# revdotcom/paper_accurate_fast_cheap

Measured on AMD Instinct MI355X. Metric: audio-sec/sec (1/RTF) GigaSpeech long-form encode, higher is better.
Workload: dtype f32+bf16-slot

## Files before the change

### paper_accurate_fast_cheap_amd/csrc/glue.hip

```cpp
#include <stdlib.h>

#include <type_traits>

#include "pafc_common.h"
#include "../../include/pafc_encoder_ops.h"

namespace pafc {

struct SplitBf16 {};
template <> struct Elem<SplitBf16> {
    __device__ static __forceinline__ float round(float v) { return v; }
};

namespace {

constexpr int VEC = 8;
constexpr int MAXIT = 2;

__device__ __forceinline__ void store8_split(bf16_t *hi_p, bf16_t *lo_p, const float *f) {
    float lo[VEC];
#pragma unroll
    for (int e = 0; e < VEC; ++e) lo[e] = f[e] - round_bf16(f[e]);
    store8<bf16_t>(hi_p, f);
    store8<bf16_t>(lo_p, lo);
// ... 137 lines not shown

template <typename ET>
__global__ __launch_bounds__(256) void tmix_shift_mix_kernel(int T, int C, long rows, int ndir, int rev0,
                                                             const ET *__restrict__ x, const ET *__restrict__ maa0,
                                                             const ET *__restrict__ maa1, ET *__restrict__ out,
                                                             const ET *__restrict__ prev) {
    const long gid = (long)blockIdx.x * 256 + threadIdx.x;
    const int cpr = C / VEC;
    const long row = gid / cpr;
    if (row >= rows) return;
    const int c = (int)(gid % cpr) * VEC;
    const int t = (int)(row % T);
    float xc[VEC], xp[VEC], xn[VEC];
    load8<ET>(x + row * C + c, xc);
#pragma unroll
    for (int e = 0; e < VEC; ++e) { xp[e] = 0.f; xn[e] = 0.f; }
    if (t > 0) load8<ET>(x + (row - 1) * C + c, xp);
    else if (prev) load8<ET>(prev + (row / T) * C + c, xp);
    if (t < T - 1) load8<ET>(x + (row + 1) * C + c, xn);
    for (int d = 0; d < ndir; ++d) {
        const bool rev = (d == 0) ? (rev0 != 0) : true;
        float m[VEC], o[VEC];
        load8<ET>((d == 0 ? maa0 : maa1) + c, m);
#pragma unroll
        for (int e = 0; e < VEC; ++e) {
            const float xx = Elem<ET>::round((rev ? xn[e] : xp[e]) - xc[e]);
            o[e] = Elem<ET>::round(xc[e] + Elem<ET>::round(xx * m[e]));
        }
        store8<ET>(out + ((size_t)d * rows + row) * C + c, o);
    }
}

template <typename ET>
__global__ __launch_bounds__(256) void tmix_mix4_kernel(int T, int C, long rows, int ndir, int rev0,
                                                        const ET *__restrict__ x, const ET *__restrict__ m,
                                                        const ET *__restrict__ maa, ET *__restrict__ z) {
    const long gid = (long)blockIdx.x * 256 + threadIdx.x;
    const int cpr = C / VEC;
    const long row = gid / cpr;
    if (row >= rows) return;
    const int c = (int)(gid % cpr) * VEC;
    const int t = (int)(row % T);
    float xc[VEC], xp[VEC], xn[VEC];
    load8<ET>(x + row * C + c, xc);
#pragma unroll
    for (int e = 0; e < VEC; ++e) { xp[e] = 0.f; xn[e] = 0.f; }
    if (t > 0) load8<ET>(x + (row - 1) * C + c, xp);
    if (t < T - 1) load8<ET>(x + (row + 1) * C + c, xn);
    for (int d = 0; d < ndir; ++d) {
        const bool rev = (d == 0) ? (rev0 != 0) : true;
        float xx[VEC];
#pragma unroll
        for (int e = 0; e < VEC; ++e) xx[e] = Elem<ET>::round((rev ? xn[e] : xp[e]) - xc[e]);
#pragma unroll
        for (int q = 0; q < 4; ++q) {
            float mv[VEC], av[VEC], o[VEC];
            load8<ET>(m + (((size_t)d * 4 + q) * rows + row) * C + c, mv);
            load8<ET>(maa + ((size_t)d * 4 + q) * C + c, av);
#pragma unroll
            for (int e = 0; e < VEC; ++e)
                o[e] = Elem<ET>::round(xc[e] + Elem<ET>::round(xx[e] * Elem<ET>::round(av[e] + mv[e])));
            store8<ET>(z + (((size_t)q * ndir + d) * rows + row) * C + c, o);
        }
    }
}

template <bool LDSW, bool FULLROW = false>
__global__ __launch_bounds__(256) void tmix_lora_mix4_kernel(int T, int C, long rows, int ndir, int rev0,
                                                             const bf16_t *__restrict__ x, const bf16_t *__restrict__ t,
                                                             const bf16_t *__restrict__ w2t,
                                                             const bf16_t *__restrict__ maa, bf16_t *__restrict__ z,
                                                             const bf16_t *__restrict__ prev) {
    const int lane = threadIdx.x & 63, wave = threadIdx.x >> 6;
    const int r16 = lane & 15, qq = lane >> 4;
    const long row = ((long)blockIdx.x * 4 + wave) * 16 + r16;
    const long rowc = row < rows ? row : rows - 1;
    const int tt = (int)(rowc % T);
    const f32x4 zero = {0.f, 0.f, 0.f, 0.f};
    constexpr int LDZ = 64 + 8;
    __shared__ __attribute__((aligned(16))) bf16_t s_z[4][16][LDZ];
    __shared__ __attribute__((aligned(16))) bf16_t s_w2[LDSW ? 2 : 1][LDSW ? 4 : 1][LDSW ? 64 : 1][32];
    if constexpr (LDSW) {
        for (int i = threadIdx.x; i < ndir * 4 * 64 * 4; i += 256) {
            const int ck = i & 3, col = (i >> 2) & 63, dq = i >> 8;
            *reinterpret_cast<uint4 *>(&s_w2[0][0][0][0] + ((size_t)dq * 64 + col) * 32 + 8 * ck) =
                *reinterpret_cast<const uint4 *>(w2t + ((size_t)dq * C + blockIdx.y * 64 + col) * 32 + 8 * ck);
        }
        __syncthreads();
    }
    for (int d = 0; d < ndir; ++d) {
        const bool rev = (d == 0) ? (rev0 != 0) : true;
        const bool in_seq = rev ? (tt < T - 1) : (tt > 0);
        const bool has_nb = in_seq || (prev != nullptr && !rev);
        const bf16_t *nbrow = in_seq ? x + (rev ? rowc + 1 : rowc - 1) * C : (has_nb ? prev + (rowc / T) * C : x + rowc * C);
        uint4 tb[4];
#pragma unroll
        for (int q = 0; q < 4; ++q)
            tb[q] = *reinterpret_cast<const uint4 *>(t + ((size_t)d * rows + rowc) * 128 + 32 * q + 8 * qq);
        float xc[2][VEC], xx[2][VEC];
#pragma unroll
        for (int cbi = 0; cbi < 2; ++cbi) {
            const int col = (blockIdx.y * 2 + cbi) * 32 + 8 * qq;
            float xn[VEC];
            load8<bf16_t>(x + rowc * C + col, xc[cbi]);
            load8<bf16_t>(nbrow + col, xn);
#pragma unroll
            for (int e = 0; e < VEC; ++e) xx[cbi][e] = round_bf16((has_nb ? xn[e] : 0.f) - xc[cbi][e]);
        }
#pragma unroll
        for (int q = 0; q < 4; ++q) {
#pragma unroll
            for (int cbi = 0; cbi < 2; ++cbi) {
                const int cb = blockIdx.y * 2 + cbi;
                const int col = cb * 32 + 8 * qq;
                const int colA = cb * 32 + 8 * (r16 >> 2) + (r16 & 3);
                uint4 a1, a2;
                if constexpr (LDSW) {
                    const int colL = colA - blockIdx.y * 64;
                    a1 = *reinterpret_cast<const uint4 *>(&s_w2[d][q][colL][8 * qq]);
                    a2 = *reinterpret_cast<const uint4 *>(&s_w2[d][q][colL + 4][8 * qq]);
                } else {
                    const bf16_t *wq = w2t + ((size_t)(d * 4 + q) * C) * 32 + 8 * qq;
                    a1 = *reinterpret_cast<const uint4 *>(wq + (size_t)colA * 32);
                    a2 = *reinterpret_cast<const uint4 *>(wq + (size_t)(colA + 4) * 32);
                }
                const f32x4 m1 = mfma_bf16_packed(a1, tb[q], zero);
                const f32x4 m2 = mfma_bf16_packed(a2, tb[q], zero);
                float av[VEC], o[VEC];
                load8<bf16_t>(maa + ((size_t)d * 4 + q) * C + col, av);
#pragma unroll
                for (int e = 0; e < VEC; ++e) {
                    const float mv = round_bf16(e < 4 ? m1[e] : m2[e - 4]);
                    o[e] = round_bf16(xc[cbi][e] + round_bf16(xx[cbi][e] * round_bf16(av[e] + mv)));
                }
                store8<bf16_t>(&s_z[wave][r16][cbi * 32 + 8 * qq], o);
            }
            __builtin_amdgcn_fence(__ATOMIC_RELEASE, "wavefront");
            __builtin_amdgcn_wave_barrier();
#pragma unroll
            for (int half = 0; half < 2; ++half) {
                const int rr = half * 8 + (lane >> 3), cc = (lane & 7) * 8;
                const long orow = ((long)blockIdx.x * 4 + wave) * 16 + rr;
                if (orow < rows)
                    *reinterpret_cast<uint4 *>(z + (((size_t)q * ndir + d) * rows + orow) * C + blockIdx.y * 64 + cc) =
                        *reinterpret_cast<const uint4 *>(&s_z[wave][rr][cc]);
            }
            __builtin_amdgcn_fence(__ATOMIC_RELEASE, "wavefront");
            __builtin_amdgcn_wave_barrier();
        }
    }
}


template <int NW, int WCOLS>
__global__ __launch_bounds__(NW * 64) void tmix_lora_mix4_ws_kernel(int T, int C, long rows, int ndir, int rev0,
                                                                const bf16_t *__restrict__ x, const bf16_t *__restrict__ t,
                                                                const bf16_t *__restrict__ w2t,
                                                                const bf16_t *__restrict__ maa, bf16_t *__restrict__ z,
                                                                const bf16_t *__restrict__ prev) {
    const int lane = threadIdx.x & 63, wave = threadIdx.x >> 6;
    const int r16 = lane & 15, qq = lane >> 4;
    constexpr int WROWS = NW / WCOLS;
    const int cy = blockIdx.y * WCOLS + wave % WCOLS, d = blockIdx.z;
    const int wrow = wave / WCOLS;
    const bool rev = (d == 0) ? (rev0 != 0) : true;
    const f32x4 zero = {0.f, 0.f, 0.f, 0.f};
    constexpr int LDZ = 64 + 8;
    __shared__ __attribute__((aligned(16))) bf16_t s_z[NW][16][LDZ];
    const int colslot = 8 * (r16 >> 2) + (r16 & 3);
    uint4 a1[4][2], a2[4][2], av[4][2];
#pragma unroll
    for (int q = 0; q < 4; ++q)
#pragma unroll
        for (int cbi = 0; cbi < 2; ++cbi) {
            const int cb = cy * 2 + cbi;
            const bf16_t *wq = w2t + ((size_t)(d * 4 + q) * C + cb * 32 + colslot) * 32 + 8 * qq;
            a1[q][cbi] = *reinterpret_cast<const uint4 *>(wq);
            a2[q][cbi] = *reinterpret_cast<const uint4 *>(wq + 4 * 32);
            av[q][cbi] = *reinterpret_cast<const uint4 *>(maa + ((size_t)d * 4 + q) * C + cb * 32 + 8 * qq);
        }
    const long ntiles = (rows + 15) / 16;
    for (long tile = (long)blockIdx.x * WROWS + wrow; tile < ntiles; tile += (long)gridDim.x * WROWS) {
        const long row = tile * 16 + r16;
        const long rowc = row < rows ? row : rows - 1;
        const int tt = (int)(rowc % T);
        const bool in_seq = rev ? (tt < T - 1) : (tt > 0);
        const bool has_nb = in_seq || (prev != nullptr && !rev);
        const bf16_t *nbrow = in_seq ? x + (rev ? rowc + 1 : rowc - 1) * C : (has_nb ? prev + (rowc / T) * C : x + rowc * C);
        uint4 tb[4];
#pragma unroll
        for (int q = 0; q < 4; ++q)
            tb[q] = *reinterpret_cast<const uint4 *>(t + ((size_t)d * rows + rowc) * 128 + 32 * q + 8 * qq);
        float xc[2][VEC], xx[2][VEC];
#pragma unroll
        for (int cbi = 0; cbi < 2; ++cbi) {
            const int col = (cy * 2 + cbi) * 32 + 8 * qq;
            float xn[VEC];
            load8<bf16_t>(x + rowc * C + col, xc[cbi]);
            load8<bf16_t>(nbrow + col, xn);
#pragma unroll
            for (int e = 0; e < VEC; ++e) xx[cbi][e] = round_bf16((has_nb ? xn[e] : 0.f) - xc[cbi][e]);
        }
#pragma unroll
        for (int q = 0; q < 4; ++q) {
#pragma unroll
            for (int cbi = 0; cbi < 2; ++cbi) {
                const f32x4 m1 = mfma_bf16_packed(a1[q][cbi], tb[q], zero);
                const f32x4 m2 = mfma_bf16_packed(a2[q][cbi], tb[q], zero);
                const unsigned aw[4] = {av[q][cbi].x, av[q][cbi].y, av[q][cbi].z, av[q][cbi].w};
                float o[VEC];
#pragma unroll
                for (int e = 0; e < VEC; ++e) {
                    const float a = (e & 1) ? __uint_as_float(aw[e >> 1] & 0xffff0000u) : __uint_as_float(aw[e >> 1] << 16);
                    const float mv = round_bf16(e < 4 ? m1[e] : m2[e - 4]);
                    o[e] = round_bf16(xc[cbi][e] + round_bf16(xx[cbi][e] * round_bf16(a + mv)));
                }
                store8<bf16_t>(&s_z[wave][r16][cbi * 32 + 8 * qq], o);
            }
            __builtin_amdgcn_fence(__ATOMIC_RELEASE, "wavefront");
            __builtin_amdgcn_wave_barrier();
#pragma unroll
            for (int half = 0; half < 2; ++half) {
                const int rr = half * 8 + (lane >> 3), cc = (lane & 7) * 8;
                const long orow = tile * 16 + rr;
                if (orow < rows)
                    *reinterpret_cast<uint4 *>(z + (((size_t)q * ndir + d) * rows + orow) * C + cy * 64 + cc) =
                        *reinterpret_cast<const uint4 *>(&s_z[wave][rr][cc]);
            }
            __builtin_amdgcn_fence(__ATOMIC_RELEASE, "wavefront");
            __builtin_amdgcn_wave_barrier();
        }
    }
}

constexpr int DL_C = 512, DL_H = 64;
constexpr int DL_WAVES = 8;
__global__ __launch_bounds__(DL_WAVES * 64) void decay_lora_kernel(long rows, int ndir, const bf16_t *__restrict__ zw,
                                                                   const bf16_t *__restrict__ d1n,
                                                                   const bf16_t *__restrict__ d2n,
                                                                   const bf16_t *__restrict__ bias, bf16_t *__restrict__ wout) {
    constexpr int C = DL_C;
    const int lane = threadIdx.x & 63, wave = threadIdx.x >> 6;
    const int r16 = lane & 15, qq = lane >> 4;
    const f32x4 zero = {0.f, 0.f, 0.f, 0.f};
    constexpr int LDZ = 64 + 8;
    extern __shared__ __attribute__((aligned(16))) unsigned char dl_lds[];
    uint4 *s_d1 = reinterpret_cast<uint4 *>(dl_lds);
    uint4 *s_d2 = s_d1 + 16 * 4 * 64;
    bf16_t(*s_z)[16][LDZ] = reinterpret_cast<bf16_t(*)[16][LDZ]>(s_d2 + 16 * 2 * 2 * 64);
    const int colslot = 8 * (r16 >> 2) + (r16 & 3);
    const long ntiles = (rows + 15) / 16;
    {
        const int d = blockIdx.y;
        for (int f = wave; f < 64; f += DL_WAVES) {
            const int ks = f >> 2, tau = f & 3;
            s_d1[f * 64 + lane] = *reinterpret_cast<const uint4 *>(d1n + ((size_t)d * DL_H + 16 * tau + r16) * C + 32 * ks + 8 * qq);
        }
        for (int f = wave; f < 64; f += DL_WAVES) {
            const int cb = f >> 2, a = (f >> 1) & 1, p = f & 1;
            const bf16_t *dq = d2n + ((size_t)d * C + cb * 32 + colslot + 4 * a) * DL_H + 32 * p + 4 * qq;
            const uint2 lo = *reinterpret_cast<const uint2 *>(dq), hi = *reinterpret_cast<const uint2 *>(dq + 16);
            s_d2[f * 64 + lane] = uint4{lo.x, lo.y, hi.x, hi.y};
        }
        __syncthreads();
        for (long tile = (long)blockIdx.x * DL_WAVES + wave; tile < ntiles; tile += (long)gridDim.x * DL_WAVES) {
            const long row = tile * 16 + r16;
            const long rowc = row < rows ? row : rows - 1;
            const bf16_t *zr = zw + ((size_t)d * rows + rowc) * C + 8 * qq;
            uint4 zf[16];
#pragma unroll
            for (int ks = 0; ks < 16; ++ks) zf[ks] = *reinterpret_cast<const uint4 *>(zr + 32 * ks);
            f32x4 acc1[4] = {zero, zero, zero, zero};
#pragma unroll
            for (int ks = 0; ks < 16; ++ks)
#pragma unroll
                for (int tau = 0; tau < 4; ++tau)
                    acc1[tau] = mfma_bf16_packed(s_d1[(ks * 4 + tau) * 64 + lane], zf[ks], acc1[tau]);
            u32x4 b2[2];
#pragma unroll
            for (int p = 0; p < 2; ++p) {
                float v[8];
#pragma unroll
                for (int e = 0; e < 8; ++e) v[e] = round_bf16(epilogue_act<2>(acc1[2 * p + (e >> 2)][e & 3]));
                b2[p] = u32x4{pack_bf16_exact(v[0], v[1]), pack_bf16_exact(v[2], v[3]),
                              pack_bf16_exact(v[4], v[5]), pack_bf16_exact(v[6], v[7])};
            }
            for (int cy = 0; cy < C / 64; ++cy) {
#pragma unroll
                for (int cbi = 0; cbi < 2; ++cbi) {
                    const int cb = cy * 2 + cbi;
                    f32x4 o[2];
#pragma unroll
                    for (int a = 0; a < 2; ++a) {
                        o[a] = mfma_bf16_packed(s_d2[((cb * 2 + a) * 2 + 0) * 64 + lane], b2[0], zero);
                        o[a] = mfma_bf16_packed(s_d2[((cb * 2 + a) * 2 + 1) * 64 + lane], b2[1], o[a]);
                    }
                    float ov[VEC];
#pragma unroll
                    for (int e = 0; e < VEC; ++e) ov[e] = e < 4 ? o[0][e] : o[1][e - 4];
                    if (bias) {
                        float bv[VEC];
                        load8<bf16_t>(bias + (size_t)d * C + cb * 32 + 8 * qq, bv);
#pragma unroll
                        for (int e = 0; e < VEC; ++e) ov[e] = bv[e] + round_bf16(ov[e]);
                    }
                    store8<bf16_t>(&s_z[wave][r16][cbi * 32 + 8 * qq], ov);
                }
                __builtin_amdgcn_fence(__ATOMIC_RELEASE, "wavefront");
                __builtin_amdgcn_wave_barrier();
#pragma unroll
                for (int half = 0; half < 2; ++half) {
                    const int rr = half * 8 + (lane >> 3), cc = (lane & 7) * 8;
                    const long orow = tile * 16 + rr;
                    if (orow < rows)
                        *reinterpret_cast<uint4 *>(wout + ((size_t)d * rows + orow) * C + cy * 64 + cc) =
                            *reinterpret_cast<const uint4 *>(&s_z[wave][rr][cc]);
                }
                __builtin_amdgcn_fence(__ATOMIC_RELEASE, "wavefront");
                __builtin_amdgcn_wave_barrier();
            }
        }
    }
}

constexpr int LD_C = 512, LD_N = 128;
template <int NW>
__global__ __launch_bounds__(NW * 64) void tmix_lora_down_kernel(int T, long rows, int rev0, const bf16_t *__restrict__ x,
                                                                       const bf16_t *__restrict__ maa_x,
                                                                       const bf16_t *__restrict__ w1n, bf16_t *__restrict__ tout,
                                                                       const bf16_t *__restrict__ prev) {
    constexpr int C = LD_C;
    const int lane = threadIdx.x & 63, wave = threadIdx.x >> 6;
    const int r16 = lane & 15, qq = lane >> 4;
    const f32x4 zero = {0.f, 0.f, 0.f, 0.f};
    extern __shared__ __attribute__((aligned(16))) unsigned char dl_lds[];
    uint4 *s_w1 = reinterpret_cast<uint4 *>(dl_lds);
    const int colslot = 8 * (r16 >> 2) + (r16 & 3);
    const int d = blockIdx.y;
    const bool rev = (d == 0) ? (rev0 != 0) : true;
    for (int f = wave; f < 128; f += NW) {
        const int ks = f >> 3, np = (f >> 1) & 3, a = f & 1;
        s_w1[f * 64 + lane] = *reinterpret_cast<const uint4 *>(w1n + ((size_t)d * LD_N + 32 * np + colslot + 4 * a) * C + 32 * ks + 8 * qq);
    }
    __syncthreads();
    const long ntiles = (rows + 15) / 16;
    for (long tile = (long)blockIdx.x * NW + wave; tile < ntiles; tile += (long)gridDim.x * NW) {
        const long row = tile * 16 + r16;
        const long rowc = row < rows ? row : rows - 1;
        const int tt = (int)(rowc % T);
        const bool in_seq = rev ? (tt < T - 1) : (tt > 0);
        const bool has_nb = in_seq || (prev != nullptr && !rev);
        const bf16_t *nbrow = in_seq ? x + (rev ? rowc + 1 : rowc - 1) * C : (has_nb ? prev + (rowc / T) * C : x + rowc * C);
        const bf16_t *xr = x + rowc * C + 8 * qq, *xnr = nbrow + 8 * qq, *mr = maa_x + (size_t)d * C + 8 * qq;
        f32x4 acc[4][2];
#pragma unroll
        for (int np = 0; np < 4; ++np) { acc[np][0] = zero; acc[np][1] = zero; }
#pragma unroll 1
        for (int kc = 0; kc < 16; kc += 4)
#pragma unroll
        for (int ks = kc; ks < kc + 4; ++ks) {
            float xc[VEC], xn[VEC], mm[VEC];
            load8<bf16_t>(xr + 32 * ks, xc);
            load8<bf16_t>(xnr + 32 * ks, xn);
            load8<bf16_t>(mr + 32 * ks, mm);
            float o[VEC];
#pragma unroll
            for (int e = 0; e < VEC; ++e) {
                const float xx = round_bf16((has_nb ? xn[e] : 0.f) - xc[e]);
                o[e] = xc[e] + round_bf16(xx * mm[e]);
            }
            const u32x4 bq = {pack_bf16_rne(o[0], o[1]), pack_bf16_rne(o[2], o[3]), pack_bf16_rne(o[4], o[5]),
                              pack_bf16_rne(o[6], o[7])};
            __builtin_amdgcn_s_setprio(1);
#pragma unroll
            for (int np = 0; np < 4; ++np)
#pragma unroll
                for (int a = 0; a < 2; ++a)
                    acc[np][a] = mfma_bf16_packed(s_w1[((ks * 4 + np) * 2 + a) * 64 + lane], bq, acc[np][a]);
            __builtin_amdgcn_s_setprio(0);
        }
        if (row < rows) {
#pragma unroll
            for (int np = 0; np < 4; ++np) {
                float o[VEC];
#pragma unroll
                for (int e = 0; e < VEC; ++e) o[e] = epilogue_act<2>(e < 4 ? acc[np][0][e] : acc[np][1][e - 4]);
                store8<bf16_t>(tout + ((size_t)d * rows + row) * LD_N + 32 * np + 8 * qq, o);
            }
        }
    }
}

__global__ __launch_bounds__(256) void split_planes_kernel(long rows, int cols, const float *__restrict__ x, long ldx,
                                                           bf16_t *__restrict__ out, long ldo, long lo_off, int triple) {
    const long gid = (long)blockIdx.x * 256 + threadIdx.x;
    const int cpr = cols / VEC;
    const long row = gid / cpr;
    if (row >= rows) return;
    const int c = (int)(gid % cpr) * VEC;
    float f[VEC];
    load8<float>(x + row * ldx + c, f);
    if (triple) {
        store8<bf16_t>(out + row * ldo + c, f);
        store8_split(out + row * ldo + cols + c, out + row * ldo + 2 * cols + c, f);
    } else {
        store8_split(out + row * ldo + c, out + row * ldo + lo_off + c, f);
    }
}

template <typename EX>
int launch_ln(int dtype_out, const LnArgs &a, hipStream_t s) {
    dim3 grid((a.rows + 3) / 4), block(256);
    if (dtype_out == PAFC_BF16)
        hipLaunchKernelGGL((add_layernorm_kernel<EX, bf16_t>), grid, block, 0, s, a);
    else if (dtype_out == PAFC_SPLIT_BF16)
        hipLaunchKernelGGL((add_layernorm_kernel<EX, SplitBf16>), grid, block, 0, s, a);
    else
        hipLaunchKernelGGL((add_layernorm_kernel<EX, float>), grid, block, 0, s, a);
    return hipGetLastError() == hipSuccess ? PAFC_OK : PAFC_ERR_LAUNCH;
}

}
}

extern "C" {

int pafc_add_layernorm(int dtype, int dtype_out, int rows, int C, const void *x, const void *y, float alpha,
                       const int32_t *lens, int T, int mask_y, void *x_out, const void *gamma1, const void *beta1,
                       void *out1, long ld1, int silu1, int zero1, const void *gamma2, const void *beta2, void *out2,
                       long ld2, float eps, pafc_stream_t stream) {
    return pafc_add_layernorm_ex(dtype, dtype_out, dtype_out, rows, C, x, y, alpha, lens, T, mask_y, x_out, gamma1, beta1, out1, ld1,
                                 silu1, zero1, gamma2, beta2, out2, ld2, eps, nullptr, nullptr, stream);
}

int pafc_add_layernorm_ex(int dtype, int dtype_out, int dtype_out2, int rows, int C, const void *x, const void *y, float alpha,
                          const int32_t *lens, int T, int mask_y, void *x_out, const void *gamma1, const void *beta1,
                          void *out1, long ld1, int silu1, int zero1, const void *gamma2, const void *beta2, void *out2,
                          long ld2, float eps, float *stats_x, float *stats_out1, pafc_stream_t stream) {
    if (!x) return PAFC_ERR_NULL_POINTER;
    if (stats_out1 && !out1) return PAFC_ERR_NULL_POINTER;
    if (dtype_out2 != dtype_out && !(dtype_out == PAFC_F32 && dtype_out2 == PAFC_SPLIT_BF16)) return PAFC_ERR_DTYPE;
    if (out1 && (!gamma1 || !beta1)) return PAFC_ERR_NULL_POINTER;
    if (out2 && (!gamma2 || !beta2 || !out1)) return PAFC_ERR_NULL_POINTER;
    if (rows <= 0 || C <= 0 || C % pafc::VEC || C > 64 * pafc::VEC * pafc::MAXIT || (lens && T <= 0))
        return PAFC_ERR_BAD_DIMS;
    if (ld1 % pafc::VEC || ld2 % pafc::VEC) return PAFC_ERR_BAD_DIMS;
    if (dtype == PAFC_BF16 && dtype_out != PAFC_BF16) return PAFC_ERR_DTYPE;
    if ((dtype_out == PAFC_SPLIT_BF16 && out1 && ld1 < 2 * C) || (dtype_out2 == PAFC_SPLIT_BF16 && out2 && ld2 < 2 * C))
        return PAFC_ERR_BAD_DIMS;
    pafc::LnArgs a{x, y, alpha, lens, T, mask_y, x_out, gamma1, beta1, out1, ld1, silu1, zero1,
                   gamma2, beta2, out2, ld2, rows, C, eps, dtype_out2 != dtype_out, stats_x, stats_out1};
    hipStream_t s = (hipStream_t)stream;
    if (dtype == PAFC_BF16) return pafc::launch_ln<pafc::bf16_t>(dtype_out, a, s);
    if (dtype == PAFC_F32) return pafc::launch_ln<float>(dtype_out, a, s);
    return PAFC_ERR_DTYPE;
}

int pafc_split_planes(long rows, int cols, const float *x, long ldx, void *out, long ldo, long lo_off, int triple,
                      pafc_stream_t stream) {
    if (!x || !out) return PAFC_ERR_NULL_POINTER;
    if (rows <= 0 || cols <= 0 || cols % pafc::VEC || ldx < cols || ldx % 4) return PAFC_ERR_BAD_DIMS;
    if (triple ? ldo < 3L * cols : (lo_off < cols || ldo < lo_off + cols)) return PAFC_ERR_BAD_DIMS;
    if (ldo % pafc::VEC || lo_off % pafc::VEC || (((uintptr_t)x | (uintptr_t)out) & 15)) return PAFC_ERR_ALIGNMENT;
    const long threads = rows * (cols / pafc::VEC);
    hipLaunchKernelGGL(pafc::split_planes_kernel, dim3((unsigned)((threads + 255) / 256)), dim3(256), 0, (hipStream_t)stream, rows,
                       cols, x, ldx, (pafc::bf16_t *)out, ldo, lo_off, triple);
    return hipGetLastError() == hipSuccess ? PAFC_OK : PAFC_ERR_LAUNCH;
}

int pafc_tmix_shift_mix(int dtype, int B, int T, int C, int ndir, int reverse0, const void *x, const void *maa_x0,
                        const void *maa_x1, void *out, pafc_stream_t stream) {
    return pafc_tmix_shift_mix_prev(dtype, B, T, C, ndir, reverse0, x, maa_x0, maa_x1, nullptr, out, stream);
}

int pafc_tmix_shift_mix_prev(int dtype, int B, int T, int C, int ndir, int reverse0, const void *x, const void *maa_x0,
                             const void *maa_x1, const void *prev, void *out, pafc_stream_t stream) {
    if (!x || !maa_x0 || !out || (ndir == 2 && !maa_x1)) return PAFC_ERR_NULL_POINTER;
    if (B <= 0 || T <= 0 || C <= 0 || C % pafc::VEC || ndir < 1 || ndir > 2) return PAFC_ERR_BAD_DIMS;
    const long rows = (long)B * T;
    const long threads = rows * (C / pafc::VEC);
    dim3 grid((unsigned)((threads + 255) / 256)), block(256);
    hipStream_t s = (hipStream_t)stream;
    if (dtype == PAFC_BF16)
        hipLaunchKernelGGL(pafc::tmix_shift_mix_kernel<pafc::bf16_t>, grid, block, 0, s, T, C, rows, ndir, reverse0,
                           (const pafc::bf16_t *)x, (const pafc::bf16_t *)maa_x0, (const pafc::bf16_t *)maa_x1,
                           (pafc::bf16_t *)out, (const pafc::bf16_t *)prev);
    else if (dtype == PAFC_F32)
        hipLaunchKernelGGL(pafc::tmix_shift_mix_kernel<float>, grid, block, 0, s, T, C, rows, ndir, reverse0,
                           (const float *)x, (const float *)maa_x0, (const float *)maa_x1, (float *)out, (const float *)prev);
    else
        return PAFC_ERR_DTYPE;
    return hipGetLastError() == hipSuccess ? PAFC_OK : PAFC_ERR_LAUNCH;
}

int pafc_tmix_mix4(int dtype, int B, int T, int C, int ndir, int reverse0, const void *x, const void *m,
                   const void *maa, void *z, pafc_stream_t stream) {
    if (!x || !m || !maa || !z) return PAFC_ERR_NULL_POINTER;
    if (B <= 0 || T <= 0 || C <= 0 || C % pafc::VEC || ndir < 1 || ndir > 2) return PAFC_ERR_BAD_DIMS;
    const long rows = (long)B * T;
    const long threads = rows * (C / pafc::VEC);
    dim3 grid((unsigned)((threads + 255) / 256)), block(256);
    hipStream_t s = (hipStream_t)stream;
    if (dtype == PAFC_BF16)
        hipLaunchKernelGGL(pafc::tmix_mix4_kernel<pafc::bf16_t>, grid, block, 0, s, T, C, rows, ndir, reverse0,
                           (const pafc::bf16_t *)x, (const pafc::bf16_t *)m, (const pafc::bf16_t *)maa,
                           (pafc::bf16_t *)z);
    else if (dtype == PAFC_F32)
        hipLaunchKernelGGL(pafc::tmix_mix4_kernel<float>, grid, block, 0, s, T, C, rows, ndir, reverse0,
                           (const float *)x, (const float *)m, (const float *)maa, (float *)z);
    else
        return PAFC_ERR_DTYPE;
    return hipGetLastError() == hipSuccess ? PAFC_OK : PAFC_ERR_LAUNCH;
}


int pafc_tmix_lora_mix4_bf16(int B, int T, int C, int ndir, int reverse0, const void *x, const void *t, const void *w2t,
                             const void *maa, void *z, pafc_stream_t stream) {
    return pafc_tmix_lora_mix4_bf16_prev(B, T, C, ndir, reverse0, x, t, w2t, maa, nullptr, z, stream);
}

int pafc_tmix_lora_mix4_bf16_prev(int B, int T, int C, int ndir, int reverse0, const void *x, const void *t, const void *w2t,
                                  const void *maa, const void *prev, void *z, pafc_stream_t stream) {
    if (!x || !t || !w2t || !maa || !z) return PAFC_ERR_NULL_POINTER;
    if (B <= 0 || T <= 0 || C <= 0 || C % 64 || ndir < 1 || ndir > 2) return PAFC_ERR_BAD_DIMS;
    const long rows = (long)B * T;
    dim3 grid((unsigned)((rows + 63) / 64), C / 64), block(256);
    const char *e = getenv("PAFC_LORA_LDSW");
    const long ntiles = (rows + 15) / 16;
    if (!e && ntiles >= 256) {
        const char *g = getenv("PAFC_LORA_WS_BLOCKS");
        const char *wc = getenv("PAFC_LORA_WS_WCOLS");
        const int wcols = wc ? atoi(wc) : 1;
        long G = g ? atol(g) : 2048 / ((C / 64) * ndir);
        if (G < 1) G = 1;
#define PAFC_WS(NW, WCOLS)                                                                                               \
    hipLaunchKernelGGL((pafc::tmix_lora_mix4_ws_kernel<NW, WCOLS>), dim3((unsigned)G, (C / 64) / WCOLS, ndir), dim3(NW * 64), 0, \
                       (hipStream_t)stream, T, C, rows, ndir, reverse0, (const pafc::bf16_t *)x, (const pafc::bf16_t *)t,  \
                       (const pafc::bf16_t *)w2t, (const pafc::bf16_t *)maa, (pafc::bf16_t *)z, (const pafc::bf16_t *)prev)
        if (wcols == 8 && (C / 64) % 8 == 0) PAFC_WS(8, 8);
        else if (wcols == 4 && (C / 64) % 4 == 0) PAFC_WS(4, 4);
        else PAFC_WS(4, 1);
#undef PAFC_WS
        return hipGetLastError() == hipSuccess ? PAFC_OK : PAFC_ERR_LAUNCH;
    }
    if (e && e[0] == '1')
        hipLaunchKernelGGL(pafc::tmix_lora_mix4_kernel<true>, grid, block, 0, (hipStream_t)stream, T, C, rows, ndir, reverse0,
                           (const pafc::bf16_t *)x, (const pafc::bf16_t *)t, (const pafc::bf16_t *)w2t,
                           (const pafc::bf16_t *)maa, (pafc::bf16_t *)z, (const pafc::bf16_t *)prev);
    else
        hipLaunchKernelGGL(pafc::tmix_lora_mix4_kernel<false>, grid, block, 0, (hipStream_t)stream, T, C, rows, ndir, reverse0,
                           (const pafc::bf16_t *)x, (const pafc::bf16_t *)t, (const pafc::bf16_t *)w2t,
                           (const pafc::bf16_t *)maa, (pafc::bf16_t *)z, (const pafc::bf16_t *)prev);
    return hipGetLastError() == hipSuccess ? PAFC_OK : PAFC_ERR_LAUNCH;
}

int pafc_decay_lora_bf16(long rows, int C, int H, int ndir, const void *zw, const void *d1n, const void *d2n, const void *bias,
                         void *w, pafc_stream_t stream) {
    if (!zw || !d1n || !d2n || !w) return PAFC_ERR_NULL_POINTER;
    if (rows <= 0 || ndir < 1 || ndir > 2) return PAFC_ERR_BAD_DIMS;
    if (C != pafc::DL_C || H != pafc::DL_H) return PAFC_ERR_UNSUPPORTED;
    const size_t lds = 2 * 65536 + pafc::DL_WAVES * 16 * (64 + 8) * sizeof(pafc::bf16_t);
    if (hipFuncSetAttribute((const void *)pafc::decay_lora_kernel, hipFuncAttributeMaxDynamicSharedMemorySize, (int)lds) !=
        hipSuccess)
        return PAFC_ERR_LAUNCH;
    const long ntiles = (rows + 15) / 16;
    int cus = 0, dev = 0;
    if (hipGetDevice(&dev) != hipSuccess || hipDeviceGetAttribute(&cus, hipDeviceAttributeMultiprocessorCount, dev) != hipSuccess ||
        cus <= 0)
        return PAFC_ERR_LAUNCH;
    long grid = cus / ndir;
    if (grid > (ntiles + pafc::DL_WAVES - 1) / pafc::DL_WAVES) grid = (ntiles + pafc::DL_WAVES - 1) / pafc::DL_WAVES;
    hipLaunchKernelGGL(pafc::decay_lora_kernel, dim3((unsigned)grid, ndir), dim3(pafc::DL_WAVES * 64), lds, (hipStream_t)stream, rows, ndir,
                       (const pafc::bf16_t *)zw, (const pafc::bf16_t *)d1n, (const pafc::bf16_t *)d2n,
                       (const pafc::bf16_t *)bias, (pafc::bf16_t *)w);
    return hipGetLastError() == hipSuccess ? PAFC_OK : PAFC_ERR_LAUNCH;
}

int pafc_tmix_lora_down_bf16(int B, int T, int C, int N, int ndir, int reverse0, const void *x, const void *maa_x,
                             const void *w1n, void *t, pafc_stream_t stream) {
    return pafc_tmix_lora_down_bf16_prev(B, T, C, N, ndir, reverse0, x, maa_x, w1n, nullptr, t, stream);
}

int pafc_tmix_lora_down_bf16_prev(int B, int T, int C, int N, int ndir, int reverse0, const void *x, const void *maa_x,
                                  const void *w1n, const void *prev, void *t, pafc_stream_t stream) {
    if (!x || !maa_x || !w1n || !t) return PAFC_ERR_NULL_POINTER;
    if (B <= 0 || T <= 0 || ndir < 1 || ndir > 2) return PAFC_ERR_BAD_DIMS;
    if (C != pafc::LD_C || N != pafc::LD_N) return PAFC_ERR_UNSUPPORTED;
    const size_t lds = 2 * 65536;
    const long rows = (long)B * T, ntiles = (rows + 15) / 16;
    int cus = 0, dev = 0;
    if (hipGetDevice(&dev) != hipSuccess || hipDeviceGetAttribute(&cus, hipDeviceAttributeMultiprocessorCount, dev) != hipSuccess ||
        cus <= 0)
        return PAFC_ERR_LAUNCH;
    const char *e = getenv("PAFC_LORA_DOWN_WAVES");
    const int nw = e ? atoi(e) : 8;
    long grid = cus / ndir;
    if (grid > (ntiles + nw - 1) / nw) grid = (ntiles + nw - 1) / nw;
#define PAFC_DOWN(NW)                                                                                                      \
    do {                                                                                                                   \
        if (hipFuncSetAttribute((const void *)pafc::tmix_lora_down_kernel<NW>, hipFuncAttributeMaxDynamicSharedMemorySize,  \
                                (int)lds) != hipSuccess)                                                                   \
            return PAFC_ERR_LAUNCH;                                                                                        \
        hipLaunchKernelGGL(pafc::tmix_lora_down_kernel<NW>, dim3((unsigned)grid, ndir), dim3(NW * 64), lds, (hipStream_t)stream, T, \
                           rows, reverse0, (const pafc::bf16_t *)x, (const pafc::bf16_t *)maa_x, (const pafc::bf16_t *)w1n, \
                           (pafc::bf16_t *)t, (const pafc::bf16_t *)prev);                                                 \
    } while (0)
    if (nw == 8) PAFC_DOWN(8);
    else PAFC_DOWN(16);
#undef PAFC_DOWN
    return hipGetLastError() == hipSuccess ? PAFC_OK : PAFC_ERR_LAUNCH;
}

}
```

Baseline: 48280.

## Software-pipeline global loads across tiles in LoRA mix, decay and down kernels

Adds a PIPE template path, on by default, to three LoRA kernels. Each wave issues the global loads for its next tile (x, neighbour row, t, zw) before doing the MFMA work on the current tile, so memory latency overlaps with compute. Bias and maa vectors are staged once in LDS instead of being re-read from global memory each tile. It also adds env overrides for grid size and optional s_memtime stamp instrumentation. The cost is higher register pressure from double-buffered operands, which may lower occupancy.

```diff
diff --git a/paper_accurate_fast_cheap_amd/csrc/glue.hip b/paper_accurate_fast_cheap_amd/csrc/glue.hip
--- a/paper_accurate_fast_cheap_amd/csrc/glue.hip
+++ b/paper_accurate_fast_cheap_amd/csrc/glue.hip
@@ -313,7 +313,40 @@
 }
 
 
-template <int NW, int WCOLS>
+#ifdef PAFC_TMIX_STAMPS
+constexpr int TMIX_STAMP_TRIPS = 8;
+__device__ unsigned long long *g_tmix_stamps;
+__device__ long g_tmix_stamp_waves;
+__device__ __forceinline__ unsigned long long tmix_clk() {
+    asm volatile("" ::: "memory");
+    const unsigned long long c = __builtin_amdgcn_s_memtime();
+    asm volatile("" ::: "memory");
+    return c;
+}
+#define TMIX_ST_DECL unsigned long long st_t0 = 0, st_wait = 0, st_ar = 0, st_c = 0; int st_trip = 0;
+#define TMIX_ST_START do { st_t0 = tmix_clk(); st_wait = 0; } while (0)
+#define TMIX_ST_WAIT0 do { st_c = tmix_clk(); } while (0)
+#define TMIX_ST_WAIT1(v) do { asm volatile("" ::"v"(v)); st_wait += tmix_clk() - st_c; } while (0)
+#define TMIX_ST_ARITH do { st_ar = tmix_clk(); } while (0)
+#define TMIX_ST_END(wg)                                                                                                  \
+    do {                                                                                                                 \
+        const unsigned long long st_e = tmix_clk();                                                                      \
+        if ((threadIdx.x & 63) == 0 && st_trip < TMIX_STAMP_TRIPS && (long)(wg) < g_tmix_stamp_waves) {                  \
+            unsigned long long *st_p = g_tmix_stamps + ((size_t)(wg) * TMIX_STAMP_TRIPS + st_trip) * 4;                  \
+            st_p[0] = st_t0; st_p[1] = st_wait; st_p[2] = st_ar; st_p[3] = st_e;                                          \
+        }                                                                                                                \
+        ++st_trip;                                                                                                       \
+    } while (0)
+#else
+#define TMIX_ST_DECL
+#define TMIX_ST_START do {} while (0)
+#define TMIX_ST_WAIT0 do {} while (0)
+#define TMIX_ST_WAIT1(v) do {} while (0)
+#define TMIX_ST_ARITH do {} while (0)
+#define TMIX_ST_END(wg) do {} while (0)
+#endif
+
+template <int NW, int WCOLS, bool PIPE = true>
 __global__ __launch_bounds__(NW * 64) void tmix_lora_mix4_ws_kernel(int T, int C, long rows, int ndir, int rev0,
                                                                 const bf16_t *__restrict__ x, const bf16_t *__restrict__ t,
                                                                 const bf16_t *__restrict__ w2t,
@@ -340,28 +373,54 @@
             a2[q][cbi] = *reinterpret_cast<const uint4 *>(wq + 4 * 32);
             av[q][cbi] = *reinterpret_cast<const uint4 *>(maa + ((size_t)d * 4 + q) * C + cb * 32 + 8 * qq);
         }
-    const long ntiles = (rows + 15) / 16;
-    for (long tile = (long)blockIdx.x * WROWS + wrow; tile < ntiles; tile += (long)gridDim.x * WROWS) {
-        const long row = tile * 16 + r16;
+    const long ntiles = (rows + 15) / 16, tstride = (long)gridDim.x * WROWS;
+    auto issue_x = [&](long tl, uint4(&xo)[2], uint4(&xn)[2], bool &has_nb, const bf16_t *&trow) {
+        const long row = tl * 16 + r16;
         const long rowc = row < rows ? row : rows - 1;
         const int tt = (int)(rowc % T);
         const bool in_seq = rev ? (tt < T - 1) : (tt > 0);
-        const bool has_nb = in_seq || (prev != nullptr && !rev);
+        has_nb = in_seq || (prev != nullptr && !rev);
         const bf16_t *nbrow = in_seq ? x + (rev ? rowc + 1 : rowc - 1) * C : (has_nb ? prev + (rowc / T) * C : x + rowc * C);
-        uint4 tb[4];
-#pragma unroll
-        for (int q = 0; q < 4; ++q)
-            tb[q] = *reinterpret_cast<const uint4 *>(t + ((size_t)d * rows + rowc) * 128 + 32 * q + 8 * qq);
-        float xc[2][VEC], xx[2][VEC];
+        trow = t + ((size_t)d * rows + rowc) * 128 + 8 * qq;
 #pragma unroll
         for (int cbi = 0; cbi < 2; ++cbi) {
             const int col = (cy * 2 + cbi) * 32 + 8 * qq;
+            xo[cbi] = *reinterpret_cast<const uint4 *>(x + rowc * C + col);
+            xn[cbi] = *reinterpret_cast<const uint4 *>(nbrow + col);
+        }
+    };
+    uint4 tb[4], lxo[2], lxn[2];
+    bool lhas = false;
+    const bf16_t *trow = t;
+    TMIX_ST_DECL
+    long tile = (long)blockIdx.x * WROWS + wrow;
+    if (PIPE && tile < ntiles) {
+        issue_x(tile, lxo, lxn, lhas, trow);
+#pragma unroll
+        for (int q = 0; q < 4; ++q) tb[q] = *reinterpret_cast<const uint4 *>(trow + 32 * q);
+    }
+    for (; tile < ntiles; tile += tstride) {
+        TMIX_ST_START;
+        if (!PIPE) {
+            issue_x(tile, lxo, lxn, lhas, trow);
+#pragma unroll
+            for (int q = 0; q < 4; ++q) tb[q] = *reinterpret_cast<const uint4 *>(trow + 32 * q);
+        }
+        TMIX_ST_WAIT0;
+        TMIX_ST_WAIT1(lxo[0].x);
+        const bool has_nb = lhas;
+        float xc[2][VEC], xx[2][VEC];
+#pragma unroll
+        for (int cbi = 0; cbi < 2; ++cbi) {
             float xn[VEC];
-            load8<bf16_t>(x + rowc * C + col, xc[cbi]);
-            load8<bf16_t>(nbrow + col, xn);
+            Elem<bf16_t>::unpack(lxo[cbi], xc[cbi]);
+            Elem<bf16_t>::unpack(lxn[cbi], xn);
 #pragma unroll
             for (int e = 0; e < VEC; ++e) xx[cbi][e] = round_bf16((has_nb ? xn[e] : 0.f) - xc[cbi][e]);
         }
+        const bool more = PIPE && tile + tstride < ntiles;
+        if (more) issue_x(tile + tstride, lxo, lxn, lhas, trow);
+        TMIX_ST_ARITH;
 #pragma unroll
         for (int q = 0; q < 4; ++q) {
 #pragma unroll
@@ -378,6 +437,7 @@
                 }
                 store8<bf16_t>(&s_z[wave][r16][cbi * 32 + 8 * qq], o);
             }
+            if (more) tb[q] = *reinterpret_cast<const uint4 *>(trow + 32 * q);
             __builtin_amdgcn_fence(__ATOMIC_RELEASE, "wavefront");
             __builtin_amdgcn_wave_barrier();
 #pragma unroll
@@ -391,11 +451,13 @@
             __builtin_amdgcn_fence(__ATOMIC_RELEASE, "wavefront");
             __builtin_amdgcn_wave_barrier();
         }
+        TMIX_ST_END(((long)(blockIdx.z * gridDim.y + blockIdx.y) * gridDim.x + blockIdx.x) * NW + wave);
     }
 }
 
 constexpr int DL_C = 512, DL_H = 64;
 constexpr int DL_WAVES = 8;
+template <bool PIPE = true>
 __global__ __launch_bounds__(DL_WAVES * 64) void decay_lora_kernel(long rows, int ndir, const bf16_t *__restrict__ zw,
                                                                    const bf16_t *__restrict__ d1n,
                                                                    const bf16_t *__restrict__ d2n,
@@ -409,6 +471,7 @@
     uint4 *s_d1 = reinterpret_cast<uint4 *>(dl_lds);
     uint4 *s_d2 = s_d1 + 16 * 4 * 64;
     bf16_t(*s_z)[16][LDZ] = reinterpret_cast<bf16_t(*)[16][LDZ]>(s_d2 + 16 * 2 * 2 * 64);
+    bf16_t *s_bias = &s_z[DL_WAVES][0][0];
     const int colslot = 8 * (r16 >> 2) + (r16 & 3);
     const long ntiles = (rows + 15) / 16;
     {
@@ -423,20 +486,33 @@
             const uint2 lo = *reinterpret_cast<const uint2 *>(dq), hi = *reinterpret_cast<const uint2 *>(dq + 16);
             s_d2[f * 64 + lane] = uint4{lo.x, lo.y, hi.x, hi.y};
         }
-        __syncthreads();
-        for (long tile = (long)blockIdx.x * DL_WAVES + wave; tile < ntiles; tile += (long)gridDim.x * DL_WAVES) {
-            const long row = tile * 16 + r16;
+        const long tstride = (long)gridDim.x * DL_WAVES;
+        uint4 zf[16];
+        auto issue = [&](long tl) {
+            const long row = tl * 16 + r16;
             const long rowc = row < rows ? row : rows - 1;
             const bf16_t *zr = zw + ((size_t)d * rows + rowc) * C + 8 * qq;
-            uint4 zf[16];
 #pragma unroll
             for (int ks = 0; ks < 16; ++ks) zf[ks] = *reinterpret_cast<const uint4 *>(zr + 32 * ks);
+        };
+        TMIX_ST_DECL
+        long tile = (long)blockIdx.x * DL_WAVES + wave;
+        if (PIPE && bias && threadIdx.x < C / 8)
+            reinterpret_cast<uint4 *>(s_bias)[threadIdx.x] = reinterpret_cast<const uint4 *>(bias + (size_t)d * C)[threadIdx.x];
+        if (PIPE && tile < ntiles) issue(tile);
+        __syncthreads();
+        for (; tile < ntiles; tile += tstride) {
+            TMIX_ST_START;
+            if (!PIPE) issue(tile);
+            TMIX_ST_WAIT0;
+            TMIX_ST_WAIT1(zf[0].x);
             f32x4 acc1[4] = {zero, zero, zero, zero};
 #pragma unroll
             for (int ks = 0; ks < 16; ++ks)
 #pragma unroll
                 for (int tau = 0; tau < 4; ++tau)
                     acc1[tau] = mfma_bf16_packed(s_d1[(ks * 4 + tau) * 64 + lane], zf[ks], acc1[tau]);
+            if (PIPE && tile + tstride < ntiles) issue(tile + tstride);
             u32x4 b2[2];
 #pragma unroll
             for (int p = 0; p < 2; ++p) {
@@ -446,6 +522,7 @@
                 b2[p] = u32x4{pack_bf16_exact(v[0], v[1]), pack_bf16_exact(v[2], v[3]),
                               pack_bf16_exact(v[4], v[5]), pack_bf16_exact(v[6], v[7])};
             }
+            TMIX_ST_ARITH;
             for (int cy = 0; cy < C / 64; ++cy) {
 #pragma unroll
                 for (int cbi = 0; cbi < 2; ++cbi) {
@@ -461,7 +538,8 @@
                     for (int e = 0; e < VEC; ++e) ov[e] = e < 4 ? o[0][e] : o[1][e - 4];
                     if (bias) {
                         float bv[VEC];
-                        load8<bf16_t>(bias + (size_t)d * C + cb * 32 + 8 * qq, bv);
+                        if (PIPE) load8<bf16_t>(s_bias + cb * 32 + 8 * qq, bv);
+                        else load8<bf16_t>(bias + (size_t)d * C + cb * 32 + 8 * qq, bv);
 #pragma unroll
                         for (int e = 0; e < VEC; ++e) ov[e] = bv[e] + round_bf16(ov[e]);
                     }
@@ -480,12 +558,13 @@
                 __builtin_amdgcn_fence(__ATOMIC_RELEASE, "wavefront");
                 __builtin_amdgcn_wave_barrier();
             }
+            TMIX_ST_END(((long)blockIdx.y * gridDim.x + blockIdx.x) * DL_WAVES + wave);
         }
     }
 }
 
 constexpr int LD_C = 512, LD_N = 128;
-template <int NW>
+template <int NW, bool PIPE = true>
 __global__ __launch_bounds__(NW * 64) void tmix_lora_down_kernel(int T, long rows, int rev0, const bf16_t *__restrict__ x,
                                                                        const bf16_t *__restrict__ maa_x,
                                                                        const bf16_t *__restrict__ w1n, bf16_t *__restrict__ tout,
@@ -496,58 +575,153 @@
     const f32x4 zero = {0.f, 0.f, 0.f, 0.f};
     extern __shared__ __attribute__((aligned(16))) unsigned char dl_lds[];
     uint4 *s_w1 = reinterpret_cast<uint4 *>(dl_lds);
+    const bf16_t *s_maa = reinterpret_cast<const bf16_t *>(dl_lds + 2 * 65536);
     const int colslot = 8 * (r16 >> 2) + (r16 & 3);
     const int d = blockIdx.y;
     const bool rev = (d == 0) ? (rev0 != 0) : true;
+    const long ntiles = (rows + 15) / 16, tstride = (long)gridDim.x * NW;
+    auto tile_rows = [&](long tl, const bf16_t *&xr, const bf16_t *&xnr, bool &has_nb) {
+        const long row = tl * 16 + r16;
+        const long rowc = row < rows ? row : rows - 1;
+        const int tt = (int)(rowc % T);
+        const bool in_seq = rev ? (tt < T - 1) : (tt > 0);
+        has_nb = in_seq || (prev != nullptr && !rev);
+        const bf16_t *nbrow = in_seq ? x + (rev ? rowc + 1 : rowc - 1) * C : (has_nb ? prev + (rowc / T) * C : x + rowc * C);
+        xr = x + rowc * C + 8 * qq;
+        xnr = nbrow + 8 * qq;
+    };
+    auto kstep = [&](int ks, const float *xc, const float *xn, const float *mm, bool has_nb, f32x4(&acc)[4][2]) {
+        float o[VEC];
+#pragma unroll
+        for (int e = 0; e < VEC; ++e) {
+            const float xx = round_bf16((has_nb ? xn[e] : 0.f) - xc[e]);
+            o[e] = xc[e] + round_bf16(xx * mm[e]);
+        }
+        const u32x4 bq = {pack_bf16_rne(o[0], o[1]), pack_bf16_rne(o[2], o[3]), pack_bf16_rne(o[4], o[5]),
+                          pack_bf16_rne(o[6], o[7])};
+        __builtin_amdgcn_s_setprio(1);
+#pragma unroll
+        for (int np = 0; np < 4; ++np)
+#pragma unroll
+            for (int a = 0; a < 2; ++a)
+                acc[np][a] = mfma_bf16_packed(s_w1[((ks * 4 + np) * 2 + a) * 64 + lane], bq, acc[np][a]);
+        __builtin_amdgcn_s_setprio(0);
+    };
+    auto finish = [&](long tl, const f32x4(&acc)[4][2]) {
+        const long row = tl * 16 + r16;
+        if (row < rows) {
+#pragma unroll
+            for (int np = 0; np < 4; ++np) {
+                float o[VEC];
+#pragma unroll
+                for (int e = 0; e < VEC; ++e) o[e] = epilogue_act<2>(e < 4 ? acc[np][0][e] : acc[np][1][e - 4]);
+                store8<bf16_t>(tout + ((size_t)d * rows + row) * LD_N + 32 * np + 8 * qq, o);
+            }
+        }
+    };
+    TMIX_ST_DECL
+    long tile = (long)blockIdx.x * NW + wave;
+    constexpr int GK = NW > 8 ? 2 : 4, NG = 16 / GK;
+    static_assert(NG % 2 == 0, "the set a tile's first group lies in must not depend on the trip");
+    uint4 gx[2][GK], gn[2][GK];
+    const bf16_t *xr = x, *xnr = x;
+    bool has_nb = false;
+    if (PIPE && tile < ntiles) {
+        tile_rows(tile, xr, xnr, has_nb);
+#pragma unroll
+        for (int j = 0; j < GK; ++j) {
+            gx[0][j] = *reinterpret_cast<const uint4 *>(xr + 32 * j);
+            gn[0][j] = *reinterpret_cast<const uint4 *>(xnr + 32 * j);
+        }
+    }
     for (int f = wave; f < 128; f += NW) {
         const int ks = f >> 3, np = (f >> 1) & 3, a = f & 1;
         s_w1[f * 64 + lane] = *reinterpret_cast<const uint4 *>(w1n + ((size_t)d * LD_N + 32 * np + colslot + 4 * a) * C + 32 * ks + 8 * qq);
     }
+    if (PIPE && threadIdx.x < C / 8)
+        reinterpret_cast<uint4 *>(dl_lds + 2 * 65536)[threadIdx.x] = reinterpret_cast<const uint4 *>(maa_x + (size_t)d * C)[threadIdx.x];
     __syncthreads();
-    const long ntiles = (rows + 15) / 16;
-    for (long tile = (long)blockIdx.x * NW + wave; tile < ntiles; tile += (long)gridDim.x * NW) {
-        const long row = tile * 16 + r16;
-        const long rowc = row < rows ? row : rows - 1;
-        const int tt = (int)(rowc % T);
-        const bool in_seq = rev ? (tt < T - 1) : (tt > 0);
-        const bool has_nb = in_seq || (prev != nullptr && !rev);
-        const bf16_t *nbrow = in_seq ? x + (rev ? rowc + 1 : rowc - 1) * C : (has_nb ? prev + (rowc / T) * C : x + rowc * C);
-        const bf16_t *xr = x + rowc * C + 8 * qq, *xnr = nbrow + 8 * qq, *mr = maa_x + (size_t)d * C + 8 * qq;
-        f32x4 acc[4][2];
-#pragma unroll
-        for (int np = 0; np < 4; ++np) { acc[np][0] = zero; acc[np][1] = zero; }
+    if constexpr (PIPE) {
+        for (; tile < ntiles; tile += tstride) {
+            TMIX_ST_START;
+            const bool more = tile + tstride < ntiles;
+            const bf16_t *nxr = xr, *nxnr = xnr;
+            bool nhas = false;
+            if (more) tile_rows(tile + tstride, nxr, nxnr, nhas);
+            f32x4 acc[4][2];
+#pragma unroll
+            for (int np = 0; np < 4; ++np) { acc[np][0] = zero; acc[np][1] = zero; }
+#pragma unroll
+            for (int g = 0; g < NG; ++g) {
+                if (g < NG - 1) {
+#pragma unroll
+                    for (int j = 0; j < GK; ++j) {
+                        gx[(g + 1) & 1][j] = *reinterpret_cast<const uint4 *>(xr + 32 * (GK * (g + 1) + j));
+                        gn[(g + 1) & 1][j] = *reinterpret_cast<const uint4 *>(xnr + 32 * (GK * (g + 1) + j));
+                    }
+                } else if (more) {
+#pragma unroll
+                    for (int j = 0; j < GK; ++j) {
+                        gx[0][j] = *reinterpret_cast<const uint4 *>(nxr + 32 * j);
+                        gn[0][j] = *reinterpret_cast<const uint4 *>(nxnr + 32 * j);
+                    }
+                }
+                TMIX_ST_WAIT0;
+                TMIX_ST_WAIT1(gx[g & 1][0].x);
+#pragma unroll
+                for (int j = 0; j < GK; ++j) {
+                    const int ks = GK * g + j;
+                    float xc[VEC], xn[VEC], mm[VEC];
+                    Elem<bf16_t>::unpack(gx[g & 1][j], xc);
+                    Elem<bf16_t>::unpack(gn[g & 1][j], xn);
+                    load8<bf16_t>(s_maa + 32 * ks + 8 * qq, mm);
+                    kstep(ks, xc, xn, mm, has_nb, acc);
+                }
+            }
+            TMIX_ST_ARITH;
+            finish(tile, acc);
+            TMIX_ST_END(((long)blockIdx.y * gridDim.x + blockIdx.x) * NW + wave);
+            xr = nxr; xnr = nxnr; has_nb = nhas;
+        }
+    } else {
+        for (; tile < ntiles; tile += tstride) {
+            TMIX_ST_START;
+            tile_rows(tile, xr, xnr, has_nb);
+            const bf16_t *mr = maa_x + (size_t)d * C + 8 * qq;
+            f32x4 acc[4][2];
+#pragma unroll
+            for (int np = 0; np < 4; ++np) { acc[np][0] = zero; acc[np][1] = zero; }
 #pragma unroll 1
-        for (int kc = 0; kc < 16; kc += 4)
-#pragma unroll
-        for (int ks = kc; ks < kc + 4; ++ks) {
-            float xc[VEC], xn[VEC], mm[VEC];
-            load8<bf16_t>(xr + 32 * ks, xc);
-            load8<bf16_t>(xnr + 32 * ks, xn);
-            load8<bf16_t>(mr + 32 * ks, mm);
-            float o[VEC];
-#pragma unroll
-            for (int e = 0; e < VEC; ++e) {
-                const float xx = round_bf16((has_nb ? xn[e] : 0.f) - xc[e]);
-                o[e] = xc[e] + round_bf16(xx * mm[e]);
-            }
-            const u32x4 bq = {pack_bf16_rne(o[0], o[1]), pack_bf16_rne(o[2], o[3]), pack_bf16_rne(o[4], o[5]),
-                              pack_bf16_rne(o[6], o[7])};
-            __builtin_amdgcn_s_setprio(1);
-#pragma unroll
-            for (int np = 0; np < 4; ++np)
-#pragma unroll
-                for (int a = 0; a < 2; ++a)
-                    acc[np][a] = mfma_bf16_packed(s_w1[((ks * 4 + np) * 2 + a) * 64 + lane], bq, acc[np][a]);
-            __builtin_amdgcn_s_setprio(0);
-        }
-        if (row < rows) {
-#pragma unroll
-            for (int np = 0; np < 4; ++np) {
-                float o[VEC];
-#pragma unroll
-                for (int e = 0; e < VEC; ++e) o[e] = epilogue_act<2>(e < 4 ? acc[np][0][e] : acc[np][1][e - 4]);
-                store8<bf16_t>(tout + ((size_t)d * rows + row) * LD_N + 32 * np + 8 * qq, o);
-            }
+            for (int kc = 0; kc < 16; kc += 4) {
+#ifdef PAFC_TMIX_STAMPS
+                uint4 rx[4], rn[4], rm[4];
+#pragma unroll
+                for (int j = 0; j < 4; ++j) {
+                    rx[j] = *reinterpret_cast<const uint4 *>(xr + 32 * (kc + j));
+                    rn[j] = *reinterpret_cast<const uint4 *>(xnr + 32 * (kc + j));
+                    rm[j] = *reinterpret_cast<const uint4 *>(mr + 32 * (kc + j));
+                }
+                TMIX_ST_WAIT0;
+                TMIX_ST_WAIT1(rx[0].x);
+#endif
+#pragma unroll
+                for (int ks = kc; ks < kc + 4; ++ks) {
+                    float xc[VEC], xn[VEC], mm[VEC];
+#ifdef PAFC_TMIX_STAMPS
+                    Elem<bf16_t>::unpack(rx[ks - kc], xc);
+                    Elem<bf16_t>::unpack(rn[ks - kc], xn);
+                    Elem<bf16_t>::unpack(rm[ks - kc], mm);
+#else
+                    load8<bf16_t>(xr + 32 * ks, xc);
+                    load8<bf16_t>(xnr + 32 * ks, xn);
+                    load8<bf16_t>(mr + 32 * ks, mm);
+#endif
+                    kstep(ks, xc, xn, mm, has_nb, acc);
+                }
+            }
+            TMIX_ST_ARITH;
+            finish(tile, acc);
+            TMIX_ST_END(((long)blockIdx.y * gridDim.x + blockIdx.x) * NW + wave);
         }
     }
 }
@@ -579,6 +753,17 @@
     else
         hipLaunchKernelGGL((add_layernorm_kernel<EX, float>), grid, block, 0, s, a);
     return hipGetLastError() == hipSuccess ? PAFC_OK : PAFC_ERR_LAUNCH;
+}
+
+bool tmix_pipe() {
+    const char *e = getenv("PAFC_TMIX_PIPE");
+    return !(e && e[0] == '0');
+}
+long blocks_override(const char *name, long grid) {
+    const char *e = getenv(name);
+    if (!e) return grid;
+    const long g = atol(e);
+    return g < 1 ? 1 : (g > 65535 ? 65535 : g);
 }
 
 }
@@ -694,14 +879,21 @@
         const int wcols = wc ? atoi(wc) : 1;
         long G = g ? atol(g) : 2048 / ((C / 64) * ndir);
         if (G < 1) G = 1;
-#define PAFC_WS(NW, WCOLS)                                                                                               \
-    hipLaunchKernelGGL((pafc::tmix_lora_mix4_ws_kernel<NW, WCOLS>), dim3((unsigned)G, (C / 64) / WCOLS, ndir), dim3(NW * 64), 0, \
+        const bool pipe = pafc::tmix_pipe();
+#define PAFC_WS_(NW, WCOLS, PIPE)                                                                                        \
+    hipLaunchKernelGGL((pafc::tmix_lora_mix4_ws_kernel<NW, WCOLS, PIPE>), dim3((unsigned)G, (C / 64) / WCOLS, ndir), dim3(NW * 64), 0, \
                        (hipStream_t)stream, T, C, rows, ndir, reverse0, (const pafc::bf16_t *)x, (const pafc::bf16_t *)t,  \
                        (const pafc::bf16_t *)w2t, (const pafc::bf16_t *)maa, (pafc::bf16_t *)z, (const pafc::bf16_t *)prev)
+#define PAFC_WS(NW, WCOLS)                                                                                               \
+    do {                                                                                                                 \
+        if (pipe) PAFC_WS_(NW, WCOLS, true);                                                                             \
+        else PAFC_WS_(NW, WCOLS, false);                                                                                 \
+    } while (0)
         if (wcols == 8 && (C / 64) % 8 == 0) PAFC_WS(8, 8);
         else if (wcols == 4 && (C / 64) % 4 == 0) PAFC_WS(4, 4);
         else PAFC_WS(4, 1);
 #undef PAFC_WS
+#undef PAFC_WS_
         return hipGetLastError() == hipSuccess ? PAFC_OK : PAFC_ERR_LAUNCH;
     }
     if (e && e[0] == '1')
@@ -720,10 +912,11 @@
     if (!zw || !d1n || !d2n || !w) return PAFC_ERR_NULL_POINTER;
     if (rows <= 0 || ndir < 1 || ndir > 2) return PAFC_ERR_BAD_DIMS;
     if (C != pafc::DL_C || H != pafc::DL_H) return PAFC_ERR_UNSUPPORTED;
-    const size_t lds = 2 * 65536 + pafc::DL_WAVES * 16 * (64 + 8) * sizeof(pafc::bf16_t);
-    if (hipFuncSetAttribute((const void *)pafc::decay_lora_kernel, hipFuncAttributeMaxDynamicSharedMemorySize, (int)lds) !=
-        hipSuccess)
-        return PAFC_ERR_LAUNCH;
+    const bool pipe = pafc::tmix_pipe();
+    const size_t lds = 2 * 65536 + pafc::DL_WAVES * 16 * (64 + 8) * sizeof(pafc::bf16_t) +
+                       (pipe ? pafc::DL_C * sizeof(pafc::bf16_t) : 0);
+    const void *kernel = pipe ? (const void *)pafc::decay_lora_kernel<true> : (const void *)pafc::decay_lora_kernel<false>;
+    if (hipFuncSetAttribute(kernel, hipFuncAttributeMaxDynamicSharedMemorySize, (int)lds) != hipSuccess) return PAFC_ERR_LAUNCH;
     const long ntiles = (rows + 15) / 16;
     int cus = 0, dev = 0;
     if (hipGetDevice(&dev) != hipSuccess || hipDeviceGetAttribute(&cus, hipDeviceAttributeMultiprocessorCount, dev) != hipSuccess ||
@@ -731,9 +924,14 @@
         return PAFC_ERR_LAUNCH;
     long grid = cus / ndir;
     if (grid > (ntiles + pafc::DL_WAVES - 1) / pafc::DL_WAVES) grid = (ntiles + pafc::DL_WAVES - 1) / pafc::DL_WAVES;
-    hipLaunchKernelGGL(pafc::decay_lora_kernel, dim3((unsigned)grid, ndir), dim3(pafc::DL_WAVES * 64), lds, (hipStream_t)stream, rows, ndir,
-                       (const pafc::bf16_t *)zw, (const pafc::bf16_t *)d1n, (const pafc::bf16_t *)d2n,
-                       (const pafc::bf16_t *)bias, (pafc::bf16_t *)w);
+    grid = pafc::blocks_override("PAFC_DECAY_LORA_BLOCKS", grid);
+#define PAFC_DECAY(PIPE)                                                                                                 \
+    hipLaunchKernelGGL(pafc::decay_lora_kernel<PIPE>, dim3((unsigned)grid, ndir), dim3(pafc::DL_WAVES * 64), lds, (hipStream_t)stream, \
+                       rows, ndir, (const pafc::bf16_t *)zw, (const pafc::bf16_t *)d1n, (const pafc::bf16_t *)d2n,         \
+                       (const pafc::bf16_t *)bias, (pafc::bf16_t *)w)
+    if (pipe) PAFC_DECAY(true);
+    else PAFC_DECAY(false);
+#undef PAFC_DECAY
     return hipGetLastError() == hipSuccess ? PAFC_OK : PAFC_ERR_LAUNCH;
 }
 
@@ -747,7 +945,8 @@
     if (!x || !maa_x || !w1n || !t) return PAFC_ERR_NULL_POINTER;
     if (B <= 0 || T <= 0 || ndir < 1 || ndir > 2) return PAFC_ERR_BAD_DIMS;
     if (C != pafc::LD_C || N != pafc::LD_N) return PAFC_ERR_UNSUPPORTED;
-    const size_t lds = 2 * 65536;
+    const bool pipe = pafc::tmix_pipe();
+    const size_t lds = 2 * 65536 + (pipe ? pafc::LD_C * sizeof(pafc::bf16_t) : 0);
     const long rows = (long)B * T, ntiles = (rows + 15) / 16;
     int cus = 0, dev = 0;
     if (hipGetDevice(&dev) != hipSuccess || hipDeviceGetAttribute(&cus, hipDeviceAttributeMultiprocessorCount, dev) != hipSuccess ||
@@ -757,18 +956,25 @@
     const int nw = e ? atoi(e) : 8;
     long grid = cus / ndir;
     if (grid > (ntiles + nw - 1) / nw) grid = (ntiles + nw - 1) / nw;
+    grid = pafc::blocks_override("PAFC_LORA_DOWN_BLOCKS", grid);
+#define PAFC_DOWN_(NW, PIPE)                                                                                               \
+    do {                                                                                                                   \
+        if (hipFuncSetAttribute((const void *)pafc::tmix_lora_down_kernel<NW, PIPE>,                                       \
+                                hipFuncAttributeMaxDynamicSharedMemorySize, (int)lds) != hipSuccess)                       \
+            return PAFC_ERR_LAUNCH;                                                                                        \
+        hipLaunchKernelGGL((pafc::tmix_lora_down_kernel<NW, PIPE>), dim3((unsigned)grid, ndir), dim3(NW * 64), lds,        \
+                           (hipStream_t)stream, T, rows, reverse0, (const pafc::bf16_t *)x, (const pafc::bf16_t *)maa_x,   \
+                           (const pafc::bf16_t *)w1n, (pafc::bf16_t *)t, (const pafc::bf16_t *)prev);                      \
+    } while (0)
 #define PAFC_DOWN(NW)                                                                                                      \
     do {                                                                                                                   \
-        if (hipFuncSetAttribute((const void *)pafc::tmix_lora_down_kernel<NW>, hipFuncAttributeMaxDynamicSharedMemorySize,  \
-                                (int)lds) != hipSuccess)                                                                   \
-            return PAFC_ERR_LAUNCH;                                                                                        \
-        hipLaunchKernelGGL(pafc::tmix_lora_down_kernel<NW>, dim3((unsigned)grid, ndir), dim3(NW * 64), lds, (hipStream_t)stream, T, \
-                           rows, reverse0, (const pafc::bf16_t *)x, (const pafc::bf16_t *)maa_x, (const pafc::bf16_t *)w1n, \
-                           (pafc::bf16_t *)t, (const pafc::bf16_t *)prev);                                                 \
+        if (pipe) PAFC_DOWN_(NW, true);                                                                                    \
+        else PAFC_DOWN_(NW, false);                                                                                        \
     } while (0)
     if (nw == 8) PAFC_DOWN(8);
     else PAFC_DOWN(16);
 #undef PAFC_DOWN
+#undef PAFC_DOWN_
     return hipGetLastError() == hipSuccess ? PAFC_OK : PAFC_ERR_LAUNCH;
 }
 
```

After: 48870, median of 6. +1.2%, better.
